# Rouji/ffmpeg_distributed

Measured on AMD Instinct MI355X. Metric: encoded frames/sec (node), 4K yuv420p MJPEG q=5 at 1/2/4/8 GPUs; HBM GB/s, higher is better.
Workload: dtype u8

## Files before the change

ffmpeg_distributed_amd/csrc/api.hip:

```cpp
#include <hip/hip_runtime.h>

#include <algorithm>
#include <cctype>
#include <climits>
#include <cmath>
#include <cstdarg>
#include <cstdio>
#include <cstdlib>
#include <cstring>
#include <string>
#include <vector>

#include "mjgpu.h"
#include "jpeg_tables.h"
#include "kernels.hip"
#include "scale.hip"
#include "sws_filter.h"

using namespace mjg;

namespace {


thread_local std::string g_err = "no error";
// ... 630 lines not shown
      sg.d_fstride = (long long)c->enc_frame_bytes;
      sg.range = k.in_full_range ? 0 : (p ? 2 : 1);
      c->ps[p].copy = plane_copy && sg.sw == sg.dw && sg.sh == sg.dh;
    }
  }

  int ncu = 0, per_cu = 0;
  HIP_TRY(hipDeviceGetAttribute(&ncu, hipDeviceAttributeMultiprocessorCount, device));
  HIP_TRY(hipOccupancyMaxActiveBlocksPerMultiprocessor(
      &per_cu, (const void *)k_encode<true, kEmitDefault>, 64 * kWavesPerWg, 0));
  c->enc_grid = std::max(1, ncu * std::max(1, per_cu));
  c->enc_grid_cnt = c->enc_grid;
  c->stage_cols = (size_t)c->enc_grid * kWavesPerWg * (c->optimal ? kEmitGridMul : 1);
  return alloc_slot(c, c->slot[0]);
}

void tmark(mjg_ctx *c, Slot &S, int k, int end) {
  if (!c->timing) return;
  const bool tail = k == MJG_K_SCAN_BITS || k == MJG_K_COUNT_FF || k == MJG_K_SCAN_FF || k == MJG_K_WRITE;
  if (tail && !c->timing_detail) return;
  (void)hipEventRecord(S.ev[k][end], tail ? c->tail : S.st);
}

int launch_write(mjg_ctx *c, Slot &S, int n, bool reset_status) {
  const EncGeom &g = c->geom;
  const int gps = (g.nchunks + kChunksPerWave - 1) / kChunksPerWave, ngroups = gps * n * g.nseg;
  if (reset_status) HIP_TRY(hipMemsetAsync(S.d_status, 0, 4, c->tail));
  tmark(c, S, MJG_K_WRITE, 0);
  k_write<<<(ngroups + 3) / 4, 256, 0, c->tail>>>(
      S.d_stream, S.d_chunk_bits, S.d_chunk_off, S.d_frame_bits, S.d_ff_off, g.nchunks, gps, g.nseg, n,
      S.d_seg_size, S.d_seg_off, S.d_frame_offsets, c->d_hdr, (int)c->hdr.size(),
      c->optimal ? S.d_hdr_lens : nullptr, (int)c->dht_pos, (int)c->dht_end, S.d_dht,
      c->optimal ? S.d_dht_nval : nullptr, S.d_out, (uint64_t)S.out_cap, S.d_status);
  tmark(c, S, MJG_K_WRITE, 1);
  if (c->timing_tail && !reset_status) (void)hipEventRecord(S.ev[MJG_K_TAIL][1], c->tail);
  HIP_TRY(hipGetLastError());
  HIP_TRY(hipMemcpyAsync(S.h_sizes, S.d_frame_size, n * sizeof(uint64_t), hipMemcpyDeviceToHost,
                         c->tail));
  HIP_TRY(hipMemcpyAsync(S.h_status, S.d_status, 4, hipMemcpyDeviceToHost, c->tail));
  HIP_TRY(hipEventRecord(S.done, c->tail));
  return MJG_OK;
}


template <int MODE, bool DBG>
void launch_encode2(mjg_ctx *c, Slot &S, const SegList &enc_in, int wgs, int ntasks) {
  const EncGeom &g = c->geom;
  if (g.range_convert)
    k_encode<true, MODE, DBG><<<wgs, 64 * kWavesPerWg, 0, S.st>>>(
        enc_in, g, c->d_tabs, S.d_scratch, S.d_chunk_bits, S.d_dbg, S.d_work, ntasks, S.d_hist,
        S.d_stage_bits, S.d_syms, S.d_symn);
  else
    k_encode<false, MODE, DBG><<<wgs, 64 * kWavesPerWg, 0, S.st>>>(
// ... 183 lines not shown
  if (c->optimal) {
    tmark(c, S, MJG_K_HUFF, 0);
    HIP_TRY(hipMemsetAsync(S.d_hist, 0, (size_t)n * kFrameTabWords * 4, S.st));
    launch_encode<kCount>(c, S, enc_in, std::min(wgs, c->enc_grid_cnt), ntasks);
    HIP_TRY(hipMemsetAsync(S.d_work, 0, (size_t)kXcds * kCtrStride * 4, S.st));
    k_huff_build<<<n * 4, 64, 0, S.st>>>(S.d_hist, S.d_ftabs, S.d_dht, S.d_dht_nval);
    tmark(c, S, MJG_K_HUFF, 1);
    HIP_TRY(hipGetLastError());
  }
  tmark(c, S, MJG_K_ENCODE, 0);
  if (c->optimal)
    k_emit_syms<<<c->enc_grid * kEmitGridMul, 64 * kWavesPerWg, 0, S.st>>>(g, c->d_tabs, S.d_ftabs, S.d_syms, S.d_symn,
                                                             S.d_scratch, S.d_chunk_bits, S.d_stage_bits,
                                                                  ntasks);
  else
    launch_encode<kEmitDefault>(c, S, enc_in, wgs, ntasks);
  tmark(c, S, MJG_K_ENCODE, 1);
  HIP_TRY(hipGetLastError());
  HIP_TRY(hipEventRecord(S.enc_done, S.st));
  HIP_TRY(hipStreamWaitEvent(c->tail, S.enc_done, 0));
  if (c->timing_tail) (void)hipEventRecord(S.ev[MJG_K_TAIL][0], c->tail);
  tmark(c, S, MJG_K_SCAN_BITS, 0);
  const int ndone = 1;
  if (c->rst)
    k_scan_bits_seg<<<(nsegs + 3) / 4, 256, 0, c->tail>>>(S.d_chunk_bits, S.d_chunk_off, S.d_frame_bits,
                                                            g.nchunks, nsegs, S.d_work, S.d_status, S.d_done,
                                                            ndone);
  else
    k_scan_bits<<<n, 1024, 0, c->tail>>>(S.d_chunk_bits, S.d_chunk_off, S.d_frame_bits, g.nchunks,
                                           S.d_work, S.d_status, S.d_done, ndone);
  tmark(c, S, MJG_K_SCAN_BITS, 1);
  HIP_TRY(hipGetLastError());
  tmark(c, S, MJG_K_COUNT_FF, 0);
  const int gps = (g.nchunks + kChunksPerWave - 1) / kChunksPerWave;
  k_count_ff<<<(gps * nsegs + 3) / 4, 256, 0, c->tail>>>(S.d_scratch, S.d_chunk_bits, S.d_chunk_off,
                                                           S.d_frame_bits, S.d_group_ff, g.nchunks, gps,
                                                           gps * nsegs, S.d_stream);
  tmark(c, S, MJG_K_COUNT_FF, 1);
  HIP_TRY(hipGetLastError());
  tmark(c, S, MJG_K_SCAN_FF, 0);
  k_scan_ff<<<n, 256, 0, c->tail>>>(S.d_group_ff, S.d_ff_off, S.d_frame_bits, g.nchunks, gps, g.nseg, (int)c->hdr.size(),
                                      c->optimal ? S.d_dht_nval : nullptr, S.d_hdr_lens, S.d_seg_size,
                                      S.d_seg_off, S.d_frame_size, S.d_frame_offsets, S.d_done);
  tmark(c, S, MJG_K_SCAN_FF, 1);
  HIP_TRY(hipGetLastError());
  int rc = launch_write(c, S, n, false);
  if (rc) return rc;
  S.n = n;
  S.pending = true;
  S.njobs = 1;
  S.nsynced = 0;
  S.jf0[0] = 0;
  S.jn[0] = n;
  c->head = (c->head + 1) % kSlots;
  c->nout++;
  c->launches++;
  c->synced_since_submit = false;
  return MJG_OK;
}

// ... 364 lines not shown
```

ffmpeg_distributed_amd/csrc/kernels.hip:

```cpp
#pragma once
#include <hip/hip_runtime.h>
#include <stdint.h>

#include "jpeg_tables.h"

namespace mjg {

constexpr int kEncWavesPerEU = 3;

constexpr int kMaxBlockBits = 1664;
constexpr int kSlotWords = (64 * kMaxBlockBits + 31) / 32;

constexpr int kTabWords = 704;
constexpr float kM = 12582912.0f;
constexpr float kMc = 12599296.0f;
constexpr float kRnd = 0x1p-10f;

#define MJG_PASS2_DOT                                                  \
  {1, 1, 1, 1, 1, 1, 1, 1,                                             \
   11363, 9633, 6437, 2260, -2260, -6437, -9633, -11363,               \
   10703, 4433, -4433, -10703, -10703, -4433, 4433, 10703,             \
   9633, -2259, -11362, -6436, 6436, 11362, 2259, -9633,               \
   1, -1, -1, 1, 1, -1, -1, 1,                                         \
   6437, -11362, 2261, 9633, -9633, -2261, 11362, -6437,               \
// ... 168 lines not shown
      spilled += 32;
      room += 32;
    }
    const uint32_t sh = 32u - (uint32_t)n;
    w0 = __builtin_amdgcn_alignbit(w0, w1, sh);
    w1 = __builtin_amdgcn_alignbit(w1, w2, sh);
    w2 = __builtin_amdgcn_alignbit(w2, w3, sh);
    w3 = (w3 << n) | v;
  }
  __device__ __forceinline__ void finish() {
    bits = spilled + 128u - (uint32_t)room;
    if (bits > 128u) flush();
  }
  __device__ __forceinline__ void flush() {
    const uint32_t o = 128u - (bits - spilled), j0 = spilled >> 5, nrem = (bits - spilled + 31) >> 5;
    stage[j0 * 64] = window_word(o, w0, w1);
    if (nrem > 1) stage[(j0 + 1) * 64] = window_word(o, w1, w2);
    if (nrem > 2) stage[(j0 + 2) * 64] = window_word(o, w2, w3);
    if (nrem > 3) stage[(j0 + 3) * 64] = window_word(o, w3, 0u);
  }
};

constexpr int kStageWords = (kMaxBlockBits + 31) / 32;
constexpr int kHvWords = kStageWords < 128 ? 128 : kStageWords;

typedef short short2_t __attribute__((ext_vector_type(2)));
__device__ __forceinline__ int exact_coef(const uint32_t *pkcol, int n, const uint32_t *m2p,
                                          const int *qc) {
  const int ro = n >> 3, c = n & 7;
  const uint4 mp = *(const uint4 *)(m2p + ro * 4);
  const uint32_t m[4] = {mp.x, mp.y, mp.z, mp.w};
  int acc = (int)((ro == 0 && c != 0 ? kRow0Bias : 0u) | 0x10000u);
#pragma unroll
  for (int i = 0; i < 4; i++)
    acc = __builtin_amdgcn_sdot2(__builtin_bit_cast(short2_t, pkcol[(c * 4 + i) * 64]),
                                 __builtin_bit_cast(short2_t, m[i]), acc, false);
  const int u = acc >> 17;
  const int qm = qc[c * 8 + ro];
  return (__mul24(u, qm) + (u < 0 ? (1 << 21) - 1 - (3 << 18) : (3 << 18))) >> 21;
}

__device__ __forceinline__ uint4 zz_desc(int k, const uint32_t *tabs) {
  const int n = kZigzag[k], ro = n >> 3, c = n & 7;
  return make_uint4((ro == 0 && c != 0 ? kRow0Bias : 0u) | 0x10000u, tabs[544 + c * 8 + ro],
                    (uint32_t)ro * 16u, (uint32_t)c * 4u * 64u * 4u);
}
__device__ __forceinline__ int exact_coef_t(const uint32_t *pkcol, uint4 d, const uint32_t *m2p) {
// ... 278 lines not shown
    c.x = (uint32_t)(luma ? g.lmw : 8);
    c.y = (uint32_t)(luma ? 16 : g.cmh);
    c.z = ((d >> 3) & 1u) * 8u;
    c.w = ((d >> 4) & 1u) * 8u;
    s_bd[2 * tid] = a;
    s_bd[2 * tid + 1] = c;
  }
}

__device__ __forceinline__ void task_pos(const EncGeom &g, int t, int &frame, int &chunk, int &bbase) {
  const int seg = (int)(((unsigned long long)(uint32_t)t * g.nchunks_magic) >> 40);
  chunk = t - seg * g.nchunks;
  if (g.nseg == 1) {
    frame = seg;
    bbase = 0;
    return;
  }
  frame = (int)(((unsigned long long)(uint32_t)seg * g.nseg_magic) >> 40);
  bbase = (seg - frame * g.nseg) * g.seg_blocks;
}

constexpr int kBatch = 12;

__device__ __forceinline__ uint64_t carry_row(const uint8_t *fb, const EncGeom &g, int bbase, int chunk, int lane,
                                              const uint4 *s_bd) {
  if (chunk == 0) return 0;
  const BlockPos p = block_pos(g, bbase + chunk * 64 - 8 + (lane >> 3), s_bd);
  const uint8_t *row = fb + p.poff + (size_t)min(p.y0 + (lane & 7), p.ph - 1) * p.stride;
  if (p.x0 + 8 <= p.pw && (((uintptr_t)(row + p.x0)) & 7) == 0)
    return *(const uint64_t *)(row + p.x0);
  uint64_t w = 0;
  for (int x = 0; x < 8; x++) w |= (uint64_t)row[min(p.x0 + x, p.pw - 1)] << (8 * x);
  return w;
}

__device__ __forceinline__ int carry_finish(uint64_t w, int chunk, int lane, bool rc, const EncGeom &g,
                                            const uint32_t *desc) {
  if (chunk == 0) return 128;
  const bool chroma = desc_tab(desc[block_in_mcu(g, chunk * 64 - 8 + (lane >> 3))]) != 0;
  int sum = 0;
#pragma unroll
  for (int x = 0; x < 8; x++) {
    const int p = (int)((w >> (8 * x)) & 255u);
    sum += !rc ? p : (chroma ? range_chroma(p) : range_luma(p));
  }
  sum += __shfl_xor(sum, 1, 64);
  sum += __shfl_xor(sum, 2, 64);
  sum += __shfl_xor(sum, 4, 64);
  const int d = __shfl((sum + 32) >> 6, max(lane - 56, 0) * 8, 64);
  return lane >= 56 ? d : 128;
}

constexpr int kEmitDefault = 0, kCount = 1;
constexpr int kFrameTabWords = 544;

__device__ __forceinline__ void pack_chunk(const ShiftSink &q, bool cur_active, uint32_t *slot,
                                           uint32_t *chunk_bits_t, int lane) {
  const uint32_t incl = wave_incl_scan(q.bits, lane);
  const uint32_t off = incl - q.bits;
  const uint32_t total = lane63(incl);

  const bool has = cur_active && q.bits != 0;
  const uint32_t sft = off & 31, fw = off >> 5;
  const uint32_t lw = has ? (off + q.bits - 1) >> 5 : fw;
  uint32_t head = 0, tail = 0;
  if (has) {
    if (q.bits <= 128 && !q.staged) {
      const uint32_t t = (32u - ((off + q.bits) & 31u)) & 31u, sh = 32u - t;
      const uint32_t d[5] = {(uint32_t)((uint64_t)q.w0 >> sh),
                             (uint32_t)((((uint64_t)q.w0 << 32) | q.w1) >> sh),
                             (uint32_t)((((uint64_t)q.w1 << 32) | q.w2) >> sh),
                             (uint32_t)((((uint64_t)q.w2 << 32) | q.w3) >> sh), q.w3 << t};
      const uint32_t nmid = lw - fw;
      tail = d[4];
#pragma unroll
      for (int j = 1; j < 4; j++)
        if ((uint32_t)j < nmid) slot[lw - j] = d[4 - j];
      head = nmid == 0 ? d[4] : nmid == 1 ? d[3] : nmid == 2 ? d[2] : nmid == 3 ? d[1] : d[0];
    } else {
      const uint32_t nws = (q.bits + 31) >> 5, nw = lw - fw + 1;
      const uint32_t *stg = q.stage;
      for (uint32_t m0 = 0; m0 < nw; m0 += 8) {
        uint32_t S[9];
// ... 1 lines not shown
        for (int i = 0; i < 9; i++) {
          const uint32_t j = m0 - 1 + (uint32_t)i;
          S[i] = j < nws ? stg[j * 64] : 0u;
        }
#pragma unroll
        for (int i = 0; i < 8; i++) {
          const uint32_t m = m0 + (uint32_t)i;
          const uint32_t F = sft ? (S[i] << (32u - sft)) | (S[i + 1] >> sft) : S[i + 1];
          if (m == 0) head = F;
          if (m + 1 == nw && m > 0) tail = F;
          if (m > 0 && m + 1 < nw) slot[fw + m] = F;
        }
      }
    }
  }
  const uint32_t fprev = (uint32_t)__builtin_amdgcn_update_dpp(-1, (int)fw, 0x138, 0xf, 0xf, false);
  const uint64_t firsts = __ballot(fprev != fw);
  const uint64_t later = lane < 63 ? firsts >> (lane + 1) : 0ull;
  const int last = later ? lane + (int)__builtin_ctzll(later) : 63;
  const uint32_t H = wave_incl_scan(head, lane);
  const uint32_t grp = (uint32_t)__builtin_amdgcn_ds_bpermute(last << 2, (int)H) - H + head;
  const uint32_t gnext = (uint32_t)__builtin_amdgcn_update_dpp(0, (int)grp, 0x130, 0xf, 0xf, false);
  const uint32_t fnext = (uint32_t)__builtin_amdgcn_update_dpp(-1, (int)fw, 0x130, 0xf, 0xf, false);
  if (has) {
    if (lw > fw) slot[lw] = tail | ((lane < 63 && fnext == lw) ? gnext : 0u);
    if (sft == 0) slot[fw] = grp;
  }
  if (lane == 0) *chunk_bits_t = total;
}

template <int W>
__device__ __forceinline__ void pack_chunk_short(const ShiftSink &q, uint32_t bits, uint32_t *s_w, uint32_t *slot,
                                                 uint32_t *chunk_bits_t, int lane) {
  const uint32_t incl = wave_incl_scan(bits, lane), off = incl - bits, total = lane63(incl);
  if (bits) {
    uint32_t *d = s_w + (off >> 5);
    if (W == 32) {
      const uint64_t x = (uint64_t)q.w3 << (64u - (off & 31u) - bits);
      atomicOr(d, (uint32_t)(x >> 32));
      if ((uint32_t)x) atomicOr(d + 1, (uint32_t)x);
    } else {
      const uint64_t v = ((uint64_t)q.w2 << 32) | q.w3;
      const uint32_t sh = 96u - (off & 31u) - bits;
      const uint64_t hi = sh >= 32u ? v << (sh - 32u) : v >> (32u - sh);
      const uint32_t lo = sh >= 32u ? 0u : (uint32_t)(v << sh);
      atomicOr(d, (uint32_t)(hi >> 32));
      if ((uint32_t)hi) atomicOr(d + 1, (uint32_t)hi);
      if (lo) atomicOr(d + 2, lo);
    }
  }
  asm volatile("s_waitcnt lgkmcnt(0)" ::: "memory");
  const uint32_t nw = (total + 31u) >> 5;
#pragma unroll
  for (uint32_t w = (uint32_t)lane; w < (uint32_t)(2 * W); w += 64)
    if (w < nw) {
      slot[w] = s_w[w];
      s_w[w] = 0u;
    }
  if (lane == 0) *chunk_bits_t = total;
}

template <bool RC>
__device__ __forceinline__ uint32_t row_pass(const uint64_t (&raw)[8], int tab, const uint8_t *s_rc,
                                             uint32_t *s_pk, int lane, const float *s_lim, bool watch,
                                             bool active) {
  auto row = [&](int r, float (&o)[8]) {
    const uint32_t lo = (uint32_t)raw[r], hi = (uint32_t)(raw[r] >> 32);
    float p[8];
    p[0] = (float)((lo >> 0) & 255u);
    p[1] = (float)((lo >> 8) & 255u);
    p[2] = (float)((lo >> 16) & 255u);
    p[3] = (float)((lo >> 24) & 255u);
    p[4] = (float)((hi >> 0) & 255u);
    p[5] = (float)((hi >> 8) & 255u);
    p[6] = (float)((hi >> 16) & 255u);
    p[7] = (float)((hi >> 24) & 255u);
    float t0, t1, t2, t3;
    if (RC) {
#pragma unroll
      for (int x = 0; x < 8; x++) {
        const uint32_t a = __builtin_amdgcn_perm((uint32_t)tab, x < 4 ? lo : hi,
                                                 0x0c0c0400u | (uint32_t)(x & 3));
// ... 116 lines not shown
}

constexpr int kXcds = 8, kCtrStride = 32;
template <int NX>
struct XcdUnits {
  int j, nbatch;
  __device__ __forceinline__ int start(int x) const { return (int)(((long long)x * nbatch) / NX); }
  __device__ __forceinline__ int nw(int x, int nwg) const {
    return ((nwg - x + NX - 1) / NX) * kWavesPerWg;
  }
  __device__ __forceinline__ int next(uint32_t *ctr, int nwg) const {
    for (int k = 0; k < NX; k++) {
      const int x = (j + k) & (NX - 1), e = start(x + 1);
      const int u = start(x) + nw(x, nwg) + (int)atomicAdd(ctr + x * kCtrStride, 1u);
      if (u < e) return u;
    }
    return nbatch;
  }
};

template <bool RC, int MODE, bool DBG = false>
__global__ __launch_bounds__(64 * kWavesPerWg, MODE == kCount ? 4 : kEncWavesPerEU) void k_encode(
    const SegList frames, EncGeom g, const uint32_t *__restrict__ tabs,
    uint32_t *__restrict__ scratch, uint32_t *__restrict__ chunk_bits,
    int16_t *__restrict__ dbg_coefs, uint32_t *__restrict__ work_ctr, int ntasks,
    uint32_t *__restrict__ hist, uint32_t *__restrict__ stage_all,
    uint32_t *__restrict__ syms, uint32_t *__restrict__ symn) {
  constexpr bool EM = MODE == kEmitDefault;
  __shared__ uint32_t s_ac[EM ? 512 : 1];
  __shared__ uint32_t s_dc[EM ? 32 : 1];
  __shared__ __attribute__((aligned(16))) int32_t s_qc[64];
  __shared__ uint8_t s_zz[64];
  __shared__ uint4 s_zd[64];
  __shared__ __attribute__((aligned(16))) float s_thr[64];
  __shared__ __attribute__((aligned(16))) uint32_t s_m2[32];
  __shared__ uint8_t s_rc[RC ? 512 : 1];
  __shared__ uint32_t s_desc[8];
  __shared__ uint4 s_bd[16];
  __shared__ __attribute__((aligned(16))) float s_lim[8];
  __shared__ uint32_t s_pk_all[kWavesPerWg][32 * 64];
  __shared__ uint32_t s_hv_all[MODE == kEmitDefault ? kWavesPerWg : 1][kHvWords];
  __shared__ uint32_t s_aux_all[EM ? 1 : kWavesPerWg][EM ? 1 : kCountWords];

  const int tid = threadIdx.x, wave = __builtin_amdgcn_readfirstlane(tid >> 6), lane = tid & 63;
  if (EM) {
    for (int i = tid; i < 512; i += 64 * kWavesPerWg) s_ac[i] = tabs[i];
    if (tid < 32) s_dc[tid] = tabs[512 + tid];
// ... 32 lines not shown
  const int nwg = gridDim.x;
  int u0 = xu.start(xu.j) + (int)(blockIdx.x / NX) * kWavesPerWg + wave;
  if (u0 >= xu.start(xu.j + 1)) {
    int v = 0;
    if (lane == 0) v = xu.next(work_ctr, nwg);
    u0 = __builtin_amdgcn_readfirstlane(v);
    if (u0 >= nbatch) return;
  }
  const int nblk = g.seg_blocks;
  constexpr bool rc = RC;

  int t = u0 * kBatch, tend = min(t + kBatch, ntasks);
  uint32_t nb = 0;
  int frame, chunk, bbase;
  task_pos(g, t, frame, chunk, bbase);
  int b = chunk * 64 + lane;
  bool active = b < nblk;
  auto frame_base = [&](int f) { return seg_frame(frames, f, g.frame_stride); };
  const uint8_t *fb = frame_base(frame);
  uint64_t raw[8];
  bool fast = fetch_rows(raw, fb, ((uintptr_t)fb & 7) == 0, block_pos(g, bbase + b, s_bd), active);
  int carry = carry_finish(carry_row(fb, g, bbase, chunk, lane, s_bd), chunk, lane, rc, g, s_desc);
  uint32_t skip_st = 0xfcu;

  while (true) {
    if (t + 1 == tend && lane == 0) nb = (uint32_t)xu.next(work_ctr, nwg);
    const uint32_t dsc = s_desc[block_in_mcu(g, b)];
    const int tab = desc_tab(dsc);
    if (active && !fast) fetch_rows_edge(raw, fb, block_pos(g, bbase + b, s_bd));
    int dc = 0;
    const bool watch = skip_st != 0u || (t & 3) == 0;
    const uint32_t skip = row_pass<RC>(raw, tab, s_rc, s_pk, lane, s_lim, watch, active);
    if (watch) skip_st = skip;
    const int cur_frame = frame, cur_chunk = chunk, cur_bbase = bbase;
    const bool cur_active = active;
    int tn = t + 1;
    const bool new_batch = tn >= tend;
    if (new_batch) {
      const int nbu = __builtin_amdgcn_readfirstlane(nb);
      tn = nbu < nbatch ? nbu * kBatch : -1;
    }
    if (tn >= 0) {
      task_pos(g, tn, frame, chunk, bbase);
      b = chunk * 64 + lane;
      active = b < nblk;
      fb = frame_base(frame);
// ... 44 lines not shown
      if (tn < 0) break;
      if (new_batch) {
        carry = carry_finish(crow, chunk, lane, rc, g, s_desc);
        tend = min(tn + kBatch, ntasks);
      }
      t = tn;
      continue;
    }
    ShiftSink q;
    q.act = s_ac + tab * 256;
    q.dct = s_dc + tab * 16;
    uint32_t *stage_w = stage_all + (size_t)gw * 64 * kStageWords;
    q.stage = stage_w + lane;
    const uint64_t wide = wave_parallel_blocks(cur_active ? __popcll(mask) : 0);
    if (cur_active && !((wide >> lane) & 1ull)) {
      emit_block(s_pk + lane, mask, diff, s_zd, s_m2, q);
      q.finish();
    }
    if (wide) {
      for (uint64_t hw = wide; hw; hw &= hw - 1) {
        const int h = (int)__builtin_ctzll(hw);
        const uint32_t nb = emit_block_wave(s_pk, h, __builtin_amdgcn_readlane(diff, h),
                                            __builtin_amdgcn_readlane(tab, h), s_zd, s_m2, s_ac, s_dc,
                                            s_hv, stage_w, lane);
        if (lane == h) {
          q.bits = nb;
          q.staged = true;
        }
      }
      asm volatile("s_waitcnt vmcnt(0)" ::: "memory");
    }
    const uint32_t qbits = cur_active ? q.bits : 0u;
    if (__ballot(qbits > 32u || q.staged) == 0ull)
      pack_chunk_short<32>(q, qbits, s_hv, scratch + (size_t)t * kSlotWords, chunk_bits + t, lane);
    else if (__ballot(qbits > 64u || q.staged) == 0ull)
      pack_chunk_short<64>(q, qbits, s_hv, scratch + (size_t)t * kSlotWords, chunk_bits + t, lane);
    else
      pack_chunk(q, cur_active, scratch + (size_t)t * kSlotWords, chunk_bits + t, lane);
    if (tn < 0) break;
    if (new_batch) {
      carry = carry_finish(crow, chunk, lane, rc, g, s_desc);
      tend = min(tn + kBatch, ntasks);
    }
    t = tn;
  }
  if (MODE == kCount && aux_frame >= 0) {
    asm volatile("s_waitcnt lgkmcnt(0)" ::: "memory");
    flush_counts(s_aux, hist + (size_t)aux_frame * kFrameTabWords, lane);
  }
}

__global__ __launch_bounds__(64 * kWavesPerWg) void k_emit_syms(
    EncGeom g, const uint32_t *__restrict__ tabs, const uint32_t *__restrict__ ftabs,
    const uint32_t *__restrict__ syms, const uint32_t *__restrict__ symn, uint32_t *__restrict__ scratch,
    uint32_t *__restrict__ chunk_bits, uint32_t *__restrict__ stage_all, int ntasks) {
  __shared__ uint32_t s_aux_all[kWavesPerWg][kFrameTabWords];
  __shared__ uint32_t s_desc[8];
  const int tid = threadIdx.x, wave = __builtin_amdgcn_readfirstlane(tid >> 6), lane = tid & 63;
  if (tid < 8) s_desc[tid] = tabs[672 + tid];
  __syncthreads();
  uint32_t *s_aux = s_aux_all[wave];
// ... 30 lines not shown
    const bool active = b < g.seg_blocks;
    const int tab = desc_tab(s_desc[block_in_mcu(g, b)]);
    ShiftSink q;
    q.act = s_aux + tab * 256;
    q.dct = s_aux + 512 + tab * 16;
    q.stage = stage_all + (size_t)gw * 64 * kStageWords + lane;
    const uint32_t *rec = syms + (size_t)t * kSymCap * 64 + lane;
    for (uint32_t j0 = 0; j0 < n; j0 += 8) {
      if (j0) {
#pragma unroll
        for (int i = 0; i < 8; i++) e[i] = j0 + i < n ? rec[(j0 + i) * 64] : 0u;
      }
#pragma unroll
      for (int i = 0; i < 8; i++) {
        if (j0 + i >= n) break;
        const uint32_t v = (e[i] >> 16) & 0xffu, mant = e[i] & 0xffffu;
        if (e[i] >> 31)
          q.dc((int)v, mant);
        else
          q.ac((int)v, (int)(v & 15u), mant);
      }
    }
    q.finish();
    pack_chunk(q, active, scratch + (size_t)t * kSlotWords, chunk_bits + t, lane);
  }
}

constexpr int kDhtSlot = 16 + 256;
constexpr int kPmMax = 520;

__device__ void av_qsort_pairs(int *val, int *key, int num) {
  int stack[64][2];
  int sp = 1;
  stack[0][0] = 0;
  stack[0][1] = num - 1;
#define MJG_SWAP(a, b)                     \
  do {                                     \
    const int ia_ = (a), ib_ = (b);        \
    const int tk_ = key[ia_], tv_ = val[ia_]; \
    key[ia_] = key[ib_];                   \
    val[ia_] = val[ib_];                   \
    key[ib_] = tk_;                        \
    val[ib_] = tv_;                        \
  } while (0)
#define MJG_CMP(a, b) (key[a] - key[b])
  while (sp) {
    int start = stack[--sp][0];
// ... 190 lines not shown
  if (tid == 0) s_carry = 0;
  __syncthreads();
  for (int base = 0; base < n; base += 1024) {
    const int i = base + tid;
    const uint32_t v = i < n ? in[i] : 0u;
    const uint32_t incl = wave_incl_scan(v, lane);
    if (lane == 63) s_w[wave] = incl;
    __syncthreads();
    if (wave == 0) {
      const uint32_t t = lane < 16 ? s_w[lane] : 0u;
      const uint32_t ti = wave_incl_scan(t, lane);
      if (lane < 16) s_w[lane] = ti - t;
    }
    __syncthreads();
    const uint32_t carry = s_carry;
    if (i < n) out[i] = carry + s_w[wave] + incl - v;
    __syncthreads();
    if (tid == 1023) s_carry = carry + s_w[wave] + incl;
    __syncthreads();
  }
  return s_carry;
}

__global__ __launch_bounds__(1024) void k_scan_bits(uint32_t *__restrict__ chunk_bits,
                                                    uint32_t *__restrict__ chunk_off,
                                                    uint32_t *__restrict__ frame_bits, int nchunks,
                                                    uint32_t *__restrict__ work_ctr,
                                                    uint32_t *__restrict__ status,
                                                    uint32_t *__restrict__ done, int ndone) {
  const int f = blockIdx.x;
  __builtin_amdgcn_s_setprio(kTailPrio);
  if (f == 0 && threadIdx.x < kXcds) work_ctr[threadIdx.x * kCtrStride] = 0;
  if (f == 0 && threadIdx.x == 0) *status = 0;
  {
    const int i = f * 1024 + (int)threadIdx.x;
    if (i < ndone) done[i] = 0;
  }
  uint32_t *cb = chunk_bits + (size_t)f * nchunks;
  for (int i = threadIdx.x; i < nchunks; i += 1024) cb[i] = min(cb[i], (uint32_t)kSlotWords * 32u);
  __syncthreads();
  const uint32_t t = block_excl_scan(cb, chunk_off + (size_t)f * nchunks, nchunks);
  if (threadIdx.x == 0) frame_bits[f] = t;
}

__device__ __forceinline__ uint32_t wave_excl_scan_arr(const uint32_t *in, uint32_t *out, int n, int lane) {
  uint32_t carry = 0;
  for (int i0 = 0; i0 < n; i0 += 64) {
    const int i = i0 + lane;
    const uint32_t v = i < n ? in[i] : 0u;
    const uint32_t incl = wave_incl_scan(v, lane);
    if (i < n) out[i] = carry + incl - v;
    carry += lane63(incl);
  }
  return carry;
}

__global__ __launch_bounds__(256) void k_scan_bits_seg(uint32_t *__restrict__ chunk_bits,
                                                       uint32_t *__restrict__ chunk_off,
                                                       uint32_t *__restrict__ seg_bits, int nchunks,
                                                       int nsegs, uint32_t *__restrict__ work_ctr,
                                                       uint32_t *__restrict__ status,
                                                       uint32_t *__restrict__ done, int ndone) {
  const int sg = blockIdx.x * 4 + (threadIdx.x >> 6), lane = threadIdx.x & 63;
  __builtin_amdgcn_s_setprio(kTailPrio);
  if (blockIdx.x == 0 && threadIdx.x < kXcds) work_ctr[threadIdx.x * kCtrStride] = 0;
  if (blockIdx.x == 0 && threadIdx.x == 0) *status = 0;
  {
    const int i = blockIdx.x * 256 + (int)threadIdx.x;
    if (i < ndone) done[i] = 0;
  }
  if (sg >= nsegs) return;
  uint32_t *cb = chunk_bits + (size_t)sg * nchunks;
  for (int i = lane; i < nchunks; i += 64) cb[i] = min(cb[i], (uint32_t)kSlotWords * 32u);
  const uint32_t t = wave_excl_scan_arr(cb, chunk_off + (size_t)sg * nchunks, nchunks, lane);
  if (lane == 0) seg_bits[sg] = t;
}

constexpr int kChunksPerWave = 32;
constexpr int kTailRounds = 4;
static_assert(kChunksPerWave * kSlotWords < (1 << 17), "group word offsets are 17-bit fields");

struct GroupWords {
  int s, c0, n;
  uint32_t T;
  uint32_t k0, k1;
  uint32_t info;
  const uint32_t *slot0;
};

__device__ __forceinline__ GroupWords group_words(const uint32_t *scratch, const uint32_t *chunk_bits,
                                                  const uint32_t *chunk_off, const uint32_t *seg_bits,
                                                  int nchunks, int gps, int gi, int lane) {
  GroupWords g;
  g.s = gi / gps;
  g.c0 = (gi - g.s * gps) * kChunksPerWave;
  g.n = min(kChunksPerWave, nchunks - g.c0);
  g.T = seg_bits[g.s];
// ... 106 lines not shown
  const int wave = __builtin_amdgcn_readfirstlane(threadIdx.x >> 6), lane = threadIdx.x & 63;
  const int gi = blockIdx.x * 4 + wave;
  for (int i = lane; i < 64 * kTailRounds; i += 64) s_marks[wave][i] = 0;
  if (gi >= ngroups) return;
  const GroupWords g = group_words(scratch, chunk_bits, chunk_off, seg_bits, nchunks, gps, gi, lane);
  uint8_t *sw = (uint8_t *)(stream + (size_t)g.s * nchunks * kSlotWords);
  uint32_t cnt = 0;
  for (uint32_t kb = g.k0; kb < g.k1; kb += 64 * kTailRounds) {
    uint32_t v[kTailRounds];
    group_values<kTailRounds>(g, kb, s_marks[wave], lane, v);
#pragma unroll
    for (int i = 0; i < kTailRounds; i++) {
      const uint32_t k = kb + 64 * i + lane;
      if (k < g.k1) {
        cnt += ff_bytes(v[i]);
        *(uint32_t *)(sw + 4u * k) = v[i];
      }
    }
  }
  cnt = (uint32_t)wave_sum((int)cnt);
  if (lane == 0) group_ff[gi] = cnt;
}

__global__ __launch_bounds__(256) void k_scan_ff(const uint32_t *__restrict__ group_ff,
                                                 uint32_t *__restrict__ ff_off,
                                                 const uint32_t *__restrict__ seg_bits, int nchunks, int gps, int nseg,
                                                 int hdr_len, const uint32_t *__restrict__ dht_nval,
                                                 uint32_t *__restrict__ hdr_lens, uint32_t *__restrict__ seg_size,
                                                 uint32_t *__restrict__ seg_off, uint64_t *__restrict__ frame_size,
                                                 uint64_t *__restrict__ frame_offsets, uint32_t *__restrict__ done) {
  __shared__ uint32_t s_last;
  tail_priority(seg_bits, nchunks);
  const int f = blockIdx.x, nframes = gridDim.x, wave = threadIdx.x >> 6, lane = threadIdx.x & 63;
  uint32_t mine = 0;
  for (int si = wave; si < nseg; si += 4) {
    const size_t s = (size_t)f * nseg + si, g0 = s * gps;
    uint32_t carry = 0;
    for (int i0 = 0; i0 < gps; i0 += 64) {
      const int i = i0 + lane;
      const uint32_t v = i < gps ? group_ff[g0 + i] : 0u;
      const uint32_t incl = wave_incl_scan(v, lane);
      if (i < gps) ff_off[g0 + i] = carry + incl - v;
      carry += lane63(incl);
    }
    mine = ((seg_bits[s] + 7) >> 3) + carry + 2;
    if (nseg > 1 && lane == 0) seg_size[s] = mine;
// ... 56 lines not shown
  if (lane == 0) {
    o[0] = 0xff;
    o[1] = 0xc4;
    o[2] = (uint8_t)(len >> 8);
    o[3] = (uint8_t)len;
  }
  o += 4;
  for (int t = 0; t < 4; t++) {
    const uint8_t *src = dht + ((size_t)f * 4 + t) * kDhtSlot;
    const int n = 16 + (int)nv[t];
    if (lane == 0) o[0] = (uint8_t)(t < 2 ? t : 0x10 | (t - 2));
    for (int i = lane; i < n; i += 64) o[1 + i] = src[i];
    o += 1 + n;
  }
  const int tail = hdr_len - dht_end;
  for (int i = lane; i < tail; i += 64) o[i] = hdr[dht_end + i];
}

typedef uint32_t u32_any __attribute__((aligned(1)));

__global__ __launch_bounds__(256) void k_write(
    const uint32_t *__restrict__ stream, const uint32_t *__restrict__ chunk_bits,
    const uint32_t *__restrict__ chunk_off, const uint32_t *__restrict__ seg_bits,
    const uint32_t *__restrict__ ff_off, int nchunks, int gps, int nseg, int nframes,
    const uint32_t *__restrict__ seg_size, const uint32_t *__restrict__ seg_off,
    const uint64_t *__restrict__ frame_offsets, const uint8_t *__restrict__ hdr, int hdr_len,
    const uint32_t *__restrict__ hdr_lens, int dht_pos, int dht_end, const uint8_t *__restrict__ dht,
    const uint32_t *__restrict__ dht_nval, uint8_t *__restrict__ out, uint64_t out_cap,
    uint32_t *__restrict__ status) {
  const int wave = __builtin_amdgcn_readfirstlane(threadIdx.x >> 6), lane = threadIdx.x & 63;
  tail_priority(seg_bits, nchunks);
  const int gi = blockIdx.x * 4 + wave, ngroups = gps * nseg * nframes;
  if (gi >= ngroups) return;
  const int s = gi / gps, gx = gi - s * gps, f = s / nseg, si = s - f * nseg;
  const int c0 = gx * kChunksPerWave, cl = min(c0 + kChunksPerWave, nchunks) - 1;
  const size_t i0 = (size_t)s * nchunks;
  const uint32_t k0 = (chunk_off[i0 + c0] + 31) >> 5, k1 = (chunk_off[i0 + cl] + chunk_bits[i0 + cl] + 31) >> 5;
  const uint32_t total_bytes = (seg_bits[s] + 7) >> 3;
  const uint64_t foff = frame_offsets[f];
  if (frame_offsets[f + 1] > out_cap) {
    if (lane == 0) atomicOr(status, 1u);
    return;
  }
  const uint32_t hl = hdr_lens ? hdr_lens[f] : (uint32_t)hdr_len;
  const uint64_t sbase = foff + hl + (nseg > 1 ? seg_off[s] : 0u);
  if (si == 0 && gx == 0) write_header(out + foff, f, hdr, hdr_len, dht_pos, dht_end, dht, dht_nval, lane);
  if (gx == gps - 1 && lane == 0) {
    const uint64_t segsz = nseg > 1 ? seg_size[s] : frame_offsets[f + 1] - foff - hl;
    uint8_t *m = out + sbase + segsz - 2;
    m[0] = 0xff;
    m[1] = si == nseg - 1 ? 0xd9 : (uint8_t)(0xd0 + (si & 7));
  }
  const uint8_t *sw = (const uint8_t *)(stream + i0 * kSlotWords);
  uint8_t *ob = out + sbase + ff_off[gi];
  uint32_t carry = 0;
  for (uint32_t kb = k0; kb < k1; kb += 64 * kTailRounds) {
    uint32_t v[kTailRounds];
#pragma unroll
    for (int i = 0; i < kTailRounds; i++) v[i] = *(const uint32_t *)(sw + 4u * min(kb + 64 * i + lane, k1 - 1));
#pragma unroll
    for (int i = 0; i < kTailRounds; i++) {
      if (kb + 64 * i >= k1) break;
      const uint32_t k = kb + 64 * i + lane;
      const bool valid = k < k1;
      const uint32_t w = v[i];
      const uint32_t ff = valid ? ff_bytes(w) : 0u;
      const uint32_t incl = wave_incl_scan(ff, lane);
      uint8_t *p = ob + 4 * (size_t)k + carry + incl - ff;
      const bool last = valid && 4 * k + 4 > total_bytes;
      if (valid && ff == 0 && !last) {
        *(u32_any *)p = __builtin_bswap32(w);
      } else if (valid) {
        const uint32_t nb = min(4u, total_bytes - 4 * k);
        uint64_t X = 0;
        uint32_t len = 0;
#pragma unroll
// ... 20 lines not shown
```

Before: 226,800.

## Pack encoder output into contiguous multi-chunk runs instead of per-chunk slots

In the non-optimal encode path, each wave now bit-packs consecutive chunks of a batch into one contiguous run and records a single bit length per run, carrying partial words in LDS between chunks. The tail kernels (scan_bits, count_ff, write) then work over runs instead of individual chunks, with a new k_count_ff_runs kernel realigning each run into the stream. The aim is to shrink the number of entries scanned and the misaligned per-chunk stitching work in the tail stages. In exchange, the pack routines gain carry bookkeeping and the LDS staging buffer grows.

```diff
diff --git a/ffmpeg_distributed_amd/csrc/api.hip b/ffmpeg_distributed_amd/csrc/api.hip
--- a/ffmpeg_distributed_amd/csrc/api.hip
+++ b/ffmpeg_distributed_amd/csrc/api.hip
@@ -676,13 +676,26 @@
   (void)hipEventRecord(S.ev[k][end], tail ? c->tail : S.st);
 }
 
+struct TailGroups {
+  int unit, rps, gsz, gps;
+};
+TailGroups tail_groups(const mjg_ctx *c) {
+  TailGroups t;
+  t.unit = c->optimal ? 1 : kBatch;
+  t.rps = run_rps(c->geom.nchunks, t.unit);
+  t.gsz = c->optimal ? kChunksPerWave : kRunsPerWave;
+  t.gps = (t.rps + t.gsz - 1) / t.gsz;
+  return t;
+}
+
 int launch_write(mjg_ctx *c, Slot &S, int n, bool reset_status) {
   const EncGeom &g = c->geom;
-  const int gps = (g.nchunks + kChunksPerWave - 1) / kChunksPerWave, ngroups = gps * n * g.nseg;
+  const TailGroups tg = tail_groups(c);
+  const int gps = tg.gps, ngroups = gps * n * g.nseg;
   if (reset_status) HIP_TRY(hipMemsetAsync(S.d_status, 0, 4, c->tail));
   tmark(c, S, MJG_K_WRITE, 0);
   k_write<<<(ngroups + 3) / 4, 256, 0, c->tail>>>(
-      S.d_stream, S.d_chunk_bits, S.d_chunk_off, S.d_frame_bits, S.d_ff_off, g.nchunks, gps, g.nseg, n,
+      S.d_stream, S.d_chunk_bits, S.d_chunk_off, S.d_frame_bits, S.d_ff_off, g.nchunks, tg.rps, tg.gsz, gps, g.nseg, n,
       S.d_seg_size, S.d_seg_off, S.d_frame_offsets, c->d_hdr, (int)c->hdr.size(),
       c->optimal ? S.d_hdr_lens : nullptr, (int)c->dht_pos, (int)c->dht_end, S.d_dht,
       c->optimal ? S.d_dht_nval : nullptr, S.d_out, (uint64_t)S.out_cap, S.d_status);
@@ -912,20 +925,26 @@
   if (c->timing_tail) (void)hipEventRecord(S.ev[MJG_K_TAIL][0], c->tail);
   tmark(c, S, MJG_K_SCAN_BITS, 0);
   const int ndone = 1;
+  const TailGroups tg = tail_groups(c);
   if (c->rst)
     k_scan_bits_seg<<<(nsegs + 3) / 4, 256, 0, c->tail>>>(S.d_chunk_bits, S.d_chunk_off, S.d_frame_bits,
-                                                            g.nchunks, nsegs, S.d_work, S.d_status, S.d_done,
-                                                            ndone);
+                                                            g.nchunks, tg.rps, tg.unit, nsegs, S.d_work,
+                                                            S.d_status, S.d_done, ndone);
   else
-    k_scan_bits<<<n, 1024, 0, c->tail>>>(S.d_chunk_bits, S.d_chunk_off, S.d_frame_bits, g.nchunks,
-                                           S.d_work, S.d_status, S.d_done, ndone);
+    k_scan_bits<<<n, 1024, 0, c->tail>>>(S.d_chunk_bits, S.d_chunk_off, S.d_frame_bits, g.nchunks, tg.rps,
+                                           tg.unit, S.d_work, S.d_status, S.d_done, ndone);
   tmark(c, S, MJG_K_SCAN_BITS, 1);
   HIP_TRY(hipGetLastError());
   tmark(c, S, MJG_K_COUNT_FF, 0);
-  const int gps = (g.nchunks + kChunksPerWave - 1) / kChunksPerWave;
-  k_count_ff<<<(gps * nsegs + 3) / 4, 256, 0, c->tail>>>(S.d_scratch, S.d_chunk_bits, S.d_chunk_off,
-                                                           S.d_frame_bits, S.d_group_ff, g.nchunks, gps,
-                                                           gps * nsegs, S.d_stream);
+  const int gps = tg.gps;
+  if (tg.unit == 1)
+    k_count_ff<<<(gps * nsegs + 3) / 4, 256, 0, c->tail>>>(S.d_scratch, S.d_chunk_bits, S.d_chunk_off,
+                                                             S.d_frame_bits, S.d_group_ff, g.nchunks, gps,
+                                                             gps * nsegs, S.d_stream);
+  else
+    k_count_ff_runs<<<(gps * nsegs + 3) / 4, 256, 0, c->tail>>>(S.d_scratch, S.d_chunk_bits, S.d_chunk_off,
+                                                                  S.d_frame_bits, S.d_group_ff, g.nchunks,
+                                                                  tg.rps, gps, gps * nsegs, S.d_stream);
   tmark(c, S, MJG_K_COUNT_FF, 1);
   HIP_TRY(hipGetLastError());
   tmark(c, S, MJG_K_SCAN_FF, 0);
diff --git a/ffmpeg_distributed_amd/csrc/kernels.hip b/ffmpeg_distributed_amd/csrc/kernels.hip
--- a/ffmpeg_distributed_amd/csrc/kernels.hip
+++ b/ffmpeg_distributed_amd/csrc/kernels.hip
@@ -214,7 +214,8 @@
 };
 
 constexpr int kStageWords = (kMaxBlockBits + 31) / 32;
-constexpr int kHvWords = kStageWords < 128 ? 128 : kStageWords;
+constexpr int kHvWave = 4;
+constexpr int kHvWords = kStageWords + 2 + kHvWave < 132 ? 132 : kStageWords + 2 + kHvWave;
 
 typedef short short2_t __attribute__((ext_vector_type(2)));
 __device__ __forceinline__ int exact_coef(const uint32_t *pkcol, int n, const uint32_t *m2p,
@@ -539,6 +540,16 @@
 
 constexpr int kBatch = 12;
 
+__host__ __device__ __forceinline__ int run_rps(int nchunks, int unit) { return (nchunks + unit - 2) / unit + 1; }
+struct Run {
+  int t0, n;
+};
+__device__ __forceinline__ Run run_of(int s, int j, int nchunks, int unit) {
+  const int first = s * nchunks, a = (first / unit + j) * unit;
+  const int t0 = max(a, first);
+  return {t0, min(a + unit, first + nchunks) - t0};
+}
+
 __device__ __forceinline__ uint64_t carry_row(const uint8_t *fb, const EncGeom &g, int bbase, int chunk, int lane,
                                               const uint4 *s_bd) {
   if (chunk == 0) return 0;
@@ -571,11 +582,28 @@
 constexpr int kEmitDefault = 0, kCount = 1;
 constexpr int kFrameTabWords = 544;
 
-__device__ __forceinline__ void pack_chunk(const ShiftSink &q, bool cur_active, uint32_t *slot,
-                                           uint32_t *chunk_bits_t, int lane) {
+template <bool RUN>
+__device__ __forceinline__ uint32_t pack_chunk(const ShiftSink &q, bool cur_active, uint32_t *slot,
+                                               uint32_t base, bool end, uint32_t *s_carry,
+                                               uint32_t *chunk_bits_t, int lane) {
   const uint32_t incl = wave_incl_scan(q.bits, lane);
-  const uint32_t off = incl - q.bits;
+  const uint32_t off = (RUN ? base : 0u) + incl - q.bits;
   const uint32_t total = lane63(incl);
+  uint32_t cin = 0, pw = ~0u;
+  if (RUN) {
+    if (lane == 0) {
+      cin = s_carry[0];
+      s_carry[0] = 0u;
+    }
+    const uint32_t tot = base + total;
+    if (!end && (tot & 31u)) pw = tot >> 5;
+  }
+  auto put = [&](uint32_t i, uint32_t v) {
+    if (RUN && i == pw)
+      s_carry[0] = v;
+    else
+      slot[i] = v;
+  };
 
   const bool has = cur_active && q.bits != 0;
   const uint32_t sft = off & 31, fw = off >> 5;
@@ -623,17 +651,16 @@
   const uint32_t grp = (uint32_t)__builtin_amdgcn_ds_bpermute(last << 2, (int)H) - H + head;
   const uint32_t gnext = (uint32_t)__builtin_amdgcn_update_dpp(0, (int)grp, 0x130, 0xf, 0xf, false);
   const uint32_t fnext = (uint32_t)__builtin_amdgcn_update_dpp(-1, (int)fw, 0x130, 0xf, 0xf, false);
-  if (has) {
-    if (lw > fw) slot[lw] = tail | ((lane < 63 && fnext == lw) ? gnext : 0u);
-    if (sft == 0) slot[fw] = grp;
-  }
-  if (lane == 0) *chunk_bits_t = total;
+  if (has && lw > fw) put(lw, tail | ((lane < 63 && fnext == lw) ? gnext : 0u));
+  if ((has && sft == 0) || (RUN && lane == 0 && base != 0)) put(fw, grp | cin);
+  if (!RUN && lane == 0) *chunk_bits_t = total;
+  return total;
 }
 
 template <int W>
-__device__ __forceinline__ void pack_chunk_short(const ShiftSink &q, uint32_t bits, uint32_t *s_w, uint32_t *slot,
-                                                 uint32_t *chunk_bits_t, int lane) {
-  const uint32_t incl = wave_incl_scan(bits, lane), off = incl - bits, total = lane63(incl);
+__device__ __forceinline__ uint32_t pack_chunk_short(const ShiftSink &q, uint32_t bits, uint32_t *s_w, uint32_t *slot,
+                                                     uint32_t base, bool end, int lane) {
+  const uint32_t incl = wave_incl_scan(bits, lane), off = base + incl - bits, total = lane63(incl);
   if (bits) {
     uint32_t *d = s_w + (off >> 5);
     if (W == 32) {
@@ -651,14 +678,23 @@
     }
   }
   asm volatile("s_waitcnt lgkmcnt(0)" ::: "memory");
-  const uint32_t nw = (total + 31u) >> 5;
-#pragma unroll
-  for (uint32_t w = (uint32_t)lane; w < (uint32_t)(2 * W); w += 64)
-    if (w < nw) {
+  const uint32_t tot = base + total, nfull = tot >> 5;
+  const uint32_t nst = end ? (tot + 31u) >> 5 : nfull;
+#pragma unroll
+  for (uint32_t w0 = 0; w0 < (uint32_t)(2 * W + 1); w0 += 64) {
+    if (w0 >= nst) break;
+    const uint32_t w = w0 + (uint32_t)lane;
+    if (w < nst) {
       slot[w] = s_w[w];
       s_w[w] = 0u;
     }
-  if (lane == 0) *chunk_bits_t = total;
+  }
+  if (!end && nfull && lane == 0) {
+    const uint32_t c = s_w[nfull];
+    s_w[nfull] = 0u;
+    s_w[0] = c;
+  }
+  return total;
 }
 
 template <bool RC>
@@ -821,7 +857,7 @@
 template <bool RC, int MODE, bool DBG = false>
 __global__ __launch_bounds__(64 * kWavesPerWg, MODE == kCount ? 4 : kEncWavesPerEU) void k_encode(
     const SegList frames, EncGeom g, const uint32_t *__restrict__ tabs,
-    uint32_t *__restrict__ scratch, uint32_t *__restrict__ chunk_bits,
+    uint32_t *__restrict__ scratch, uint32_t *__restrict__ run_bits,
     int16_t *__restrict__ dbg_coefs, uint32_t *__restrict__ work_ctr, int ntasks,
     uint32_t *__restrict__ hist, uint32_t *__restrict__ stage_all,
     uint32_t *__restrict__ syms, uint32_t *__restrict__ symn) {
@@ -900,6 +936,8 @@
   bool fast = fetch_rows(raw, fb, ((uintptr_t)fb & 7) == 0, block_pos(g, bbase + b, s_bd), active);
   int carry = carry_finish(carry_row(fb, g, bbase, chunk, lane, s_bd), chunk, lane, rc, g, s_desc);
   uint32_t skip_st = 0xfcu;
+  int run_t0 = t;
+  uint32_t run_len = 0;
 
   while (true) {
     if (t + 1 == tend && lane == 0) nb = (uint32_t)xu.next(work_ctr, nwg);
@@ -990,7 +1028,7 @@
         const int h = (int)__builtin_ctzll(hw);
         const uint32_t nb = emit_block_wave(s_pk, h, __builtin_amdgcn_readlane(diff, h),
                                             __builtin_amdgcn_readlane(tab, h), s_zd, s_m2, s_ac, s_dc,
-                                            s_hv, stage_w, lane);
+                                            s_hv + kHvWave, stage_w, lane);
         if (lane == h) {
           q.bits = nb;
           q.staged = true;
@@ -999,12 +1037,23 @@
       asm volatile("s_waitcnt vmcnt(0)" ::: "memory");
     }
     const uint32_t qbits = cur_active ? q.bits : 0u;
+    const bool run_end = new_batch || cur_chunk + 1 == g.nchunks;
+    uint32_t *run_w = scratch + (size_t)run_t0 * kSlotWords + (run_len >> 5);
+    uint32_t cbits;
     if (__ballot(qbits > 32u || q.staged) == 0ull)
-      pack_chunk_short<32>(q, qbits, s_hv, scratch + (size_t)t * kSlotWords, chunk_bits + t, lane);
+      cbits = pack_chunk_short<32>(q, qbits, s_hv, run_w, run_len & 31u, run_end, lane);
     else if (__ballot(qbits > 64u || q.staged) == 0ull)
-      pack_chunk_short<64>(q, qbits, s_hv, scratch + (size_t)t * kSlotWords, chunk_bits + t, lane);
+      cbits = pack_chunk_short<64>(q, qbits, s_hv, run_w, run_len & 31u, run_end, lane);
     else
-      pack_chunk(q, cur_active, scratch + (size_t)t * kSlotWords, chunk_bits + t, lane);
+      cbits = pack_chunk<true>(q, cur_active, run_w, run_len & 31u, run_end, s_hv, nullptr, lane);
+    run_len += cbits;
+    if (run_end) {
+      const int s = t - cur_chunk, sg = (int)(((unsigned long long)(uint32_t)t * g.nchunks_magic) >> 40);
+      if (lane == 0)
+        run_bits[sg * run_rps(g.nchunks, kBatch) + run_t0 / kBatch - s / kBatch] = run_len;
+      run_len = 0;
+      run_t0 = tn;
+    }
     if (tn < 0) break;
     if (new_batch) {
       carry = carry_finish(crow, chunk, lane, rc, g, s_desc);
@@ -1081,7 +1130,7 @@
       }
     }
     q.finish();
-    pack_chunk(q, active, scratch + (size_t)t * kSlotWords, chunk_bits + t, lane);
+    pack_chunk<false>(q, active, scratch + (size_t)t * kSlotWords, 0u, true, nullptr, chunk_bits + t, lane);
   }
 }
 
@@ -1318,10 +1367,15 @@
   return s_carry;
 }
 
+__device__ __forceinline__ uint32_t run_bits_clamped(const uint32_t *rb, int s, int j, int nchunks, int unit) {
+  const Run r = run_of(s, j, nchunks, unit);
+  return r.n > 0 ? min(rb[j], (uint32_t)r.n * (uint32_t)kSlotWords * 32u) : 0u;
+}
+
 __global__ __launch_bounds__(1024) void k_scan_bits(uint32_t *__restrict__ chunk_bits,
                                                     uint32_t *__restrict__ chunk_off,
-                                                    uint32_t *__restrict__ frame_bits, int nchunks,
-                                                    uint32_t *__restrict__ work_ctr,
+                                                    uint32_t *__restrict__ frame_bits, int nchunks, int rps,
+                                                    int unit, uint32_t *__restrict__ work_ctr,
                                                     uint32_t *__restrict__ status,
                                                     uint32_t *__restrict__ done, int ndone) {
   const int f = blockIdx.x;
@@ -1332,10 +1386,10 @@
     const int i = f * 1024 + (int)threadIdx.x;
     if (i < ndone) done[i] = 0;
   }
-  uint32_t *cb = chunk_bits + (size_t)f * nchunks;
-  for (int i = threadIdx.x; i < nchunks; i += 1024) cb[i] = min(cb[i], (uint32_t)kSlotWords * 32u);
+  uint32_t *cb = chunk_bits + (size_t)f * rps;
+  for (int i = threadIdx.x; i < rps; i += 1024) cb[i] = run_bits_clamped(cb, f, i, nchunks, unit);
   __syncthreads();
-  const uint32_t t = block_excl_scan(cb, chunk_off + (size_t)f * nchunks, nchunks);
+  const uint32_t t = block_excl_scan(cb, chunk_off + (size_t)f * rps, rps);
   if (threadIdx.x == 0) frame_bits[f] = t;
 }
 
@@ -1353,8 +1407,8 @@
 
 __global__ __launch_bounds__(256) void k_scan_bits_seg(uint32_t *__restrict__ chunk_bits,
                                                        uint32_t *__restrict__ chunk_off,
-                                                       uint32_t *__restrict__ seg_bits, int nchunks,
-                                                       int nsegs, uint32_t *__restrict__ work_ctr,
+                                                       uint32_t *__restrict__ seg_bits, int nchunks, int rps,
+                                                       int unit, int nsegs, uint32_t *__restrict__ work_ctr,
                                                        uint32_t *__restrict__ status,
                                                        uint32_t *__restrict__ done, int ndone) {
   const int sg = blockIdx.x * 4 + (threadIdx.x >> 6), lane = threadIdx.x & 63;
@@ -1366,9 +1420,9 @@
     if (i < ndone) done[i] = 0;
   }
   if (sg >= nsegs) return;
-  uint32_t *cb = chunk_bits + (size_t)sg * nchunks;
-  for (int i = lane; i < nchunks; i += 64) cb[i] = min(cb[i], (uint32_t)kSlotWords * 32u);
-  const uint32_t t = wave_excl_scan_arr(cb, chunk_off + (size_t)sg * nchunks, nchunks, lane);
+  uint32_t *cb = chunk_bits + (size_t)sg * rps;
+  for (int i = lane; i < rps; i += 64) cb[i] = run_bits_clamped(cb, sg, i, nchunks, unit);
+  const uint32_t t = wave_excl_scan_arr(cb, chunk_off + (size_t)sg * rps, rps, lane);
   if (lane == 0) seg_bits[sg] = t;
 }
 
@@ -1521,6 +1575,63 @@
   if (lane == 0) group_ff[gi] = cnt;
 }
 
+constexpr int kRunsPerWave = 3;
+__global__ __launch_bounds__(256) void k_count_ff_runs(const uint32_t *__restrict__ scratch,
+                                                       const uint32_t *__restrict__ run_bits,
+                                                       const uint32_t *__restrict__ run_off,
+                                                       const uint32_t *__restrict__ seg_bits,
+                                                       uint32_t *__restrict__ group_ff, int nchunks, int rps,
+                                                       int gps, int ngroups, uint32_t *__restrict__ stream) {
+  tail_priority(seg_bits, nchunks);
+  const int wave = __builtin_amdgcn_readfirstlane(threadIdx.x >> 6), lane = threadIdx.x & 63;
+  const int gi = blockIdx.x * 4 + wave;
+  if (gi >= ngroups) return;
+  const int s = gi / gps, r0 = (gi - s * gps) * kRunsPerWave, r1 = min(r0 + kRunsPerWave, rps);
+  const uint32_t T = seg_bits[s], kT = (T + 31) >> 5;
+  const uint32_t *rb = run_bits + (size_t)s * rps, *ro = run_off + (size_t)s * rps;
+  uint32_t *sw = stream + (size_t)s * nchunks * kSlotWords;
+  uint32_t cnt = 0;
+  for (int r = r0; r < r1; r++) {
+    const uint32_t L = rb[r], O = ro[r];
+    if (L == 0) break;
+    const uint32_t ka = (O + 31) >> 5, ke = (O + L + 31) >> 5;
+    if (ka == ke) continue;
+    const uint32_t d = 32 * ka - O, nown = ke - ka, nw = (L + 31) >> 5;
+    const uint32_t *src = scratch + (size_t)run_of(s, r, nchunks, kBatch).t0 * kSlotWords;
+    const uint32_t rem = L - d - 32 * (nown - 1);
+    uint32_t extra = 0;
+    if (rem < 32u && r + 1 < rps && rb[r + 1] != 0u)
+      extra = scratch[(size_t)run_of(s, r + 1, nchunks, kBatch).t0 * kSlotWords] >> rem;
+    if (ke == kT) {
+      const uint32_t endk = T - 32 * (kT - 1), pad = (8u - (T & 7u)) & 7u;
+      if (endk < 32u) extra |= (0xffffffffu >> endk) & ~(endk + pad >= 32u ? 0u : (0xffffffffu >> (endk + pad)));
+    }
+    for (uint32_t mb = 0; mb < nown; mb += 64 * kTailRounds) {
+      uint32_t A[kTailRounds], N[kTailRounds];
+#pragma unroll
+      for (int i = 0; i < kTailRounds; i++) {
+        if (mb + 64 * i >= nown) break;
+        const uint32_t m = mb + 64 * i + lane;
+        A[i] = m < nown ? src[m] : 0u;
+        N[i] = (d != 0u && m < nown && m + 1 < nw) ? src[m + 1] : 0u;
+      }
+#pragma unroll
+      for (int i = 0; i < kTailRounds; i++) {
+        if (mb + 64 * i >= nown) break;
+        const uint32_t m = mb + 64 * i + lane;
+        if (m < nown) {
+          uint32_t w = __builtin_amdgcn_alignbit(A[i], d != 0u ? N[i] : A[i], (32u - d) & 31u);
+          if (m + 1 == nown) w |= extra;
+          cnt += ff_bytes(w);
+          sw[ka + m] = w;
+        }
+      }
+    }
+  }
+  cnt = (uint32_t)wave_sum((int)cnt);
+  if (lane == 0) group_ff[gi] = cnt;
+}
+
 __global__ __launch_bounds__(256) void k_scan_ff(const uint32_t *__restrict__ group_ff,
                                                  uint32_t *__restrict__ ff_off,
                                                  const uint32_t *__restrict__ seg_bits, int nchunks, int gps, int nseg,
@@ -1623,7 +1734,7 @@
 __global__ __launch_bounds__(256) void k_write(
     const uint32_t *__restrict__ stream, const uint32_t *__restrict__ chunk_bits,
     const uint32_t *__restrict__ chunk_off, const uint32_t *__restrict__ seg_bits,
-    const uint32_t *__restrict__ ff_off, int nchunks, int gps, int nseg, int nframes,
+    const uint32_t *__restrict__ ff_off, int nchunks, int rps, int gsz, int gps, int nseg, int nframes,
     const uint32_t *__restrict__ seg_size, const uint32_t *__restrict__ seg_off,
     const uint64_t *__restrict__ frame_offsets, const uint8_t *__restrict__ hdr, int hdr_len,
     const uint32_t *__restrict__ hdr_lens, int dht_pos, int dht_end, const uint8_t *__restrict__ dht,
@@ -1634,8 +1745,8 @@
   const int gi = blockIdx.x * 4 + wave, ngroups = gps * nseg * nframes;
   if (gi >= ngroups) return;
   const int s = gi / gps, gx = gi - s * gps, f = s / nseg, si = s - f * nseg;
-  const int c0 = gx * kChunksPerWave, cl = min(c0 + kChunksPerWave, nchunks) - 1;
-  const size_t i0 = (size_t)s * nchunks;
+  const int c0 = gx * gsz, cl = min(c0 + gsz, rps) - 1;
+  const size_t i0 = (size_t)s * rps;
   const uint32_t k0 = (chunk_off[i0 + c0] + 31) >> 5, k1 = (chunk_off[i0 + cl] + chunk_bits[i0 + cl] + 31) >> 5;
   const uint32_t total_bytes = (seg_bits[s] + 7) >> 3;
   const uint64_t foff = frame_offsets[f];
@@ -1652,7 +1763,7 @@
     m[0] = 0xff;
     m[1] = si == nseg - 1 ? 0xd9 : (uint8_t)(0xd0 + (si & 7));
   }
-  const uint8_t *sw = (const uint8_t *)(stream + i0 * kSlotWords);
+  const uint8_t *sw = (const uint8_t *)(stream + (size_t)s * nchunks * kSlotWords);
   uint8_t *ob = out + sbase + ff_off[gi];
   uint32_t carry = 0;
   for (uint32_t kb = k0; kb < k1; kb += 64 * kTailRounds) {
```

New measurement: 227,100, median of 6. No clear change (+0.1%).
